# ccw1996/Paddle_hackathon

Hardware: AMD Instinct MI355X
Metric: tokens/sec GPT-3-1.3B fleet DP (bf16, whole job) (higher is better)
Workload: dtype bf16; 1 GPU; model=GPT-3-1.3B, global_batch=48, seq_len=2048, parallelism=dp1, micro_batch_per_gpu=48, n_params=1315819520, optimizer=AdamW fp32-master

## Files before the change

paddle_hackathon_amd/csrc/kernels/ce_gelu_embed.hip:

```cpp
#include "common.h"
#include <algorithm>

using namespace pha;

namespace {

template <typename T, bool VEC = true>
__global__ __launch_bounds__(256) void softmax_ce_fwd_kernel(const T* __restrict__ logits, const int64_t* __restrict__ labels,
                                                             float* __restrict__ loss, float* __restrict__ lse_out,
                                                             int V, int ignore_index) {
  const long row = blockIdx.x;
  const T* xr = logits + row * (long)V;
  float m = -INFINITY, s = 0.f;
  if constexpr (VEC) {
    for (int c = threadIdx.x * 8; c < V; c += 256 * 8) {
      float v[8];
      Vec8<T>::ld(xr + c, v);
      float vm = v[0];
#pragma unroll
      for (int i = 1; i < 8; ++i) vm = fmaxf(vm, v[i]);
      const float nm = fmaxf(m, vm);
      float acc = s * __expf(m - nm);
#pragma unroll
      for (int i = 0; i < 8; ++i) acc += __expf(v[i] - nm);
// ... 83 lines not shown
  const float e = __expf(2.f * u);
  return 1.f - 2.f * __builtin_amdgcn_rcpf(e + 1.f);
}

__device__ __forceinline__ float gelu_f(float x, bool approx) {
  if (approx) {
    const float k = 0.7978845608028654f;
    const float u = k * (x + 0.044715f * x * x * x);
    return 0.5f * x * (1.f + fast_tanh(u));
  }
  return 0.5f * x * (1.f + erff(x * 0.7071067811865476f));
}

__device__ __forceinline__ float gelu_grad(float x, bool approx) {
  if (approx) {
    constexpr float k = 0.7978845608028654f, c = 0.044715f;
    constexpr float c0 = -2.f * k * 1.4426950408889634f, c1 = c0 * c;
    const float x2 = x * x;
    const float sg = __builtin_amdgcn_rcpf(1.f + __builtin_amdgcn_exp2f(x * __builtin_fmaf(x2, c1, c0)));
    const float q = x * __builtin_fmaf(x2, 6.f * k * c, 2.f * k) * (1.f - sg);
    return __builtin_fmaf(q, sg, sg);
  }
  const float cdf = 0.5f * (1.f + erff(x * 0.7071067811865476f));
  const float pdf = 0.3989422804014327f * __expf(-0.5f * x * x);
  return cdf + x * pdf;
}

template <typename T>
__global__ __launch_bounds__(256) void bias_gelu_fwd_kernel(const T* __restrict__ x, const T* __restrict__ b, T* __restrict__ y,
                                                            long n8, int H, bool approx) {
  for (long i = blockIdx.x * 256L + threadIdx.x; i < n8; i += (long)gridDim.x * 256) {
    float v[8], o[8];
    Vec8<T>::ld(x + i * 8, v);
    if (b) {
      float bv[8];
      Vec8<T>::ld(b + (int)((unsigned)i % (unsigned)(H / 8)) * 8, bv);
// ... 585 lines not shown
```

paddle_hackathon_amd/csrc/kernels/common.h:

```cpp
#pragma once
#include <hip/hip_runtime.h>
#include <stdint.h>

#define PHA_API extern "C" __attribute__((visibility("default")))

namespace pha {

enum DType : int { kF32 = 0, kBF16 = 1, kF16 = 2 };

struct bf16_t { uint16_t v; };
struct half_t { _Float16 v; };

__device__ __forceinline__ float bf16_to_f32(uint16_t h) {
  return __uint_as_float(static_cast<uint32_t>(h) << 16);
}
__device__ __forceinline__ uint16_t f32_to_bf16(float f) {
  uint32_t u = __float_as_uint(f);
  if ((u & 0x7fffffffu) > 0x7f800000u) return 0x7fc0;
  u += 0x7fffu + ((u >> 16) & 1u);
  return static_cast<uint16_t>(u >> 16);
}

template <typename T> struct Cvt;
template <> struct Cvt<float> {
// ... 61 lines not shown
  }
};
template <> struct Vec8<float> {
  static __device__ __forceinline__ void ld(const float* p, float (&o)[8]) {
    float4 a = *reinterpret_cast<const float4*>(p);
    float4 b = *reinterpret_cast<const float4*>(p + 4);
    o[0] = a.x; o[1] = a.y; o[2] = a.z; o[3] = a.w;
    o[4] = b.x; o[5] = b.y; o[6] = b.z; o[7] = b.w;
  }
  static __device__ __forceinline__ void st(float* p, const float (&o)[8]) {
    *reinterpret_cast<float4*>(p) = make_float4(o[0], o[1], o[2], o[3]);
    *reinterpret_cast<float4*>(p + 4) = make_float4(o[4], o[5], o[6], o[7]);
  }
};

__device__ __forceinline__ float wave_sum(float v) {
#pragma unroll
  for (int o = 32; o > 0; o >>= 1) v += __shfl_xor(v, o, 64);
  return v;
}
__device__ __forceinline__ float wave_max(float v) {
#pragma unroll
  for (int o = 32; o > 0; o >>= 1) v = fmaxf(v, __shfl_xor(v, o, 64));
  return v;
}

template <bool kMax>
__device__ __forceinline__ float block_reduce(float v, float* red) {
  const int lane = threadIdx.x & 63, wid = threadIdx.x >> 6, nw = blockDim.x >> 6;
  v = kMax ? wave_max(v) : wave_sum(v);
// ... 18 lines not shown
```

paddle_hackathon_amd/csrc/kernels/gemm4p.hip:

```cpp
#include "mfma_tile.h"
#include <type_traits>

namespace pha {
namespace g4p {

using namespace g256;

#ifndef PHA_G4P_RELG_NT
#define PHA_G4P_RELG_NT 8
#endif
#ifndef PHA_G4P_CS_SPLITLOOP
#define PHA_G4P_CS_SPLITLOOP 1
#endif
#ifndef PHA_G4P_RELG_TN
#define PHA_G4P_RELG_TN 8
#endif

enum : int {
  EPI_BIAS = 1,
  EPI_GELU = 2,
  EPI_NOSTORE = 512,
  EPI_SKIP = 128,
  EPI_STAGGER = 4096,
  EPI_ROUNDS = 8192,
  EPI_TEMPORAL = 16384,
  EPI_RSTAGE = 32768,
  EPI_EARLY = 65536,
  EPI_LATE_SHIFT = 17,
  EPI_L2ONLY = 1 << 21,
  EPI_RING = 1 << 22,
  EPI_ADEEP = 1 << 23,
  EPI_WSTAG = 1 << 24,
  EPI_KSTAG_SHIFT = 25,
  EPI_COLSUM = 1 << 27,
  EPI_SPREAD_SHIFT = 28,
// ... 41 lines not shown
               :: "v"(voff), "s"(sbase), "s"(m0) : "memory", "m0");
}
__device__ __forceinline__ void glds4(const void* src, unsigned m0) {
  asm volatile("s_mov_b32 m0, %1\n\ts_nop 0\n\tglobal_load_lds_dword %0, off"
               :: "v"(src), "s"(m0) : "memory", "m0");
}

__device__ __forceinline__ void bar() {
  asm volatile("" ::: "memory");
  __builtin_amdgcn_s_barrier();
  asm volatile("" ::: "memory");
}

typedef unsigned u32x4v __attribute__((ext_vector_type(4)));

__device__ __forceinline__ float gelu_t(float x) {
  constexpr float c0 = -2.f * 0.7978845608028654f * 1.4426950408889634f;
  constexpr float c1 = c0 * 0.044715f;
  const float arg = x * __builtin_fmaf(x * x, c1, c0);
  return x * __builtin_amdgcn_rcpf(__builtin_amdgcn_exp2f(arg) + 1.f);
}

template <typename T>
__device__ __forceinline__ unsigned pk(float lo, float hi) {
  if constexpr (std::is_same<T, bf16_t>::value) {
    typedef __bf16 bf2 __attribute__((ext_vector_type(2)));
    return __builtin_bit_cast(unsigned, bf2{(__bf16)lo, (__bf16)hi});
  } else {
    typedef _Float16 h2 __attribute__((ext_vector_type(2)));
    return __builtin_bit_cast(unsigned, h2{(_Float16)lo, (_Float16)hi});
  }
}

template <typename T>
__device__ __forceinline__ void mma0(f32x4& d, const uint4& a, const uint4& b) {
// ... 26 lines not shown
    const int item = c0 + r * step;
    int lin = item / splits;
    slice = __builtin_amdgcn_readfirstlane(item - lin * splits);
    bi = __builtin_amdgcn_readfirstlane(lin / per_batch);
    lin -= bi * per_batch;
    const int group = lin / (gm * tiles_n);
    const int first_m = group * gm;
    const int gsize = min(tiles_m - first_m, gm);
    const int in = lin - group * gm * tiles_n;
    tm = __builtin_amdgcn_readfirstlane(first_m + in % gsize);
    tn = __builtin_amdgcn_readfirstlane(in / gsize);
  }
};

template <typename T, bool AKO, bool BKO, bool OT, bool BIAS, bool SKIPEPI = false, bool SPLIT = false,
          bool GELU = false, bool RS = false, bool EARLY = false, int LV = 0, bool CS = false>
__global__ __launch_bounds__(256) __attribute__((amdgpu_waves_per_eu(1, 1))) void gemm4p_kernel(Args p) {
  __shared__ __attribute__((aligned(1024))) unsigned char smem[SMEM];
  const int tid = threadIdx.x, lane = tid & 63;
  const int wid = __builtin_amdgcn_readfirstlane(tid >> 6);
  const int wr = wid >> 1, wc = wid & 1;
  const int M = p.M, N = p.N, K = p.K;
  const int nsplit = SPLIT ? p.splits : 1;
  const int nk = (K >> 6) / nsplit;

  Sched sc;
  sc.tiles_m = (M + 255) >> 8;
  sc.tiles_n = (N + 255) >> 8;
  sc.splits = nsplit;
  sc.per_batch = sc.tiles_m * sc.tiles_n;
  sc.total = sc.per_batch * nsplit * p.batch;
  sc.G = gridDim.x;
// ... 135 lines not shown
  const int lcol4 = wc * 128 + 4 * fk;
  const unsigned lane_voff4 = (unsigned)(fr * ldc2 + lcol4 * 4);
  const char* e_base = static_cast<const char*>(p.c);
  const char* e_aux = static_cast<const char*>(p.aux);
  int e_rows = 0, e_cols = 0, e_slot = 0;
  auto set_epi = [&](int r) {
    int tm, tn, slice, bi;
    sc.tile(r, tm, tn, slice, bi);
    const int r0 = OT ? tn << 8 : tm << 8, c0 = OT ? tm << 8 : tn << 8;
    e_slot = r & 3;
    if constexpr (SPLIT)
      e_base = reinterpret_cast<const char*>(p.ws) + (size_t)slice * Mo * No * 4 +
               ((size_t)(r0 + wrow) * ldc2 + (size_t)c0 * 4);
    else
      e_base = static_cast<const char*>(p.c) + (size_t)bi * p.sc * 2 + ((size_t)(r0 + wrow) * ldc2 + (size_t)c0 * 2);
    if constexpr (GELU) e_aux = static_cast<const char*>(p.aux) + ((size_t)(r0 + wrow) * ldc2 + (size_t)c0 * 2);
    e_rows = (p.epi & EPI_NOSTORE) ? 0 : Mo - r0 - wrow;
    e_cols = No - c0;
  };
  auto store_pair = [&](const f32x4& x0, const f32x4& x1, int rb, int cb) {
    float v0[4], v1[4];
    asm volatile("v_accvgpr_read_b32 %0, %4\n\tv_accvgpr_read_b32 %1, %5\n\tv_accvgpr_read_b32 %2, %6\n\t"
                 "v_accvgpr_read_b32 %3, %7"
                 : "=v"(v0[0]), "=v"(v0[1]), "=v"(v0[2]), "=v"(v0[3]) : "a"(x0[0]), "a"(x0[1]), "a"(x0[2]), "a"(x0[3]));
    asm volatile("v_accvgpr_read_b32 %0, %4\n\tv_accvgpr_read_b32 %1, %5\n\tv_accvgpr_read_b32 %2, %6\n\t"
                 "v_accvgpr_read_b32 %3, %7"
                 : "=v"(v1[0]), "=v"(v1[1]), "=v"(v1[2]), "=v"(v1[3]) : "a"(x1[0]), "a"(x1[1]), "a"(x1[2]), "a"(x1[3]));
    const int nbytes = __builtin_amdgcn_readfirstlane(max(min(e_rows - rb * 16, 16), 0) * ldc2);
    const unsigned voff = (lcol + cb * 16 < e_cols) ? lane_voff : 0x80000000u;
    typedef unsigned u32x4 __attribute__((ext_vector_type(4)));
    auto pack_swap = [&](const float (&a)[4], const float (&b)[4]) {
      unsigned q00 = pk<T>(a[0], a[1]), q01 = pk<T>(a[2], a[3]);
      unsigned q10 = pk<T>(b[0], b[1]), q11 = pk<T>(b[2], b[3]);
      const auto s0 = __builtin_amdgcn_permlane16_swap(q00, q10, false, false);
      const auto s1 = __builtin_amdgcn_permlane16_swap(q01, q11, false, false);
      return u32x4{s0[0], s1[0], s0[1], s1[1]};
    };
    auto rsrc = [&](const char* base) {
      const size_t bp = (size_t)(base + (size_t)rb * 16 * ldc2);
      const unsigned blo = __builtin_amdgcn_readfirstlane((unsigned)bp);
      const unsigned bhi = __builtin_amdgcn_readfirstlane((unsigned)(bp >> 32));
      return __builtin_amdgcn_make_buffer_rsrc(reinterpret_cast<void*>(((size_t)bhi << 32) | blo), (short)0, nbytes,
                                               0x00020000);
    };
    if constexpr (GELU)
      __builtin_amdgcn_raw_buffer_store_b128(pack_swap(v0, v1), rsrc(e_aux), voff + cb * 32, 0, 2);
    if constexpr (BIAS) {
      const unsigned char* bs = smem + BIAS_OFF + e_slot * 1024 + (OT ? wr : wc) * 512 + 16 * fk;
      const f32x4 b0 = *reinterpret_cast<const f32x4*>(bs + cb * 64);
      const f32x4 b1 = *reinterpret_cast<const f32x4*>(bs + cb * 64 + 64);
#pragma unroll
      for (int e = 0; e < 4; ++e) {
        v0[e] += b0[e];
        v1[e] += b1[e];
      }
    }
    if constexpr (GELU) {
#pragma unroll
      for (int e = 0; e < 4; ++e) {
        v0[e] = gelu_t(v0[e]);
        v1[e] = gelu_t(v1[e]);
      }
    }
    const auto rs = rsrc(e_base);
    const u32x4 q = pack_swap(v0, v1);
    if (p.epi & EPI_TEMPORAL) __builtin_amdgcn_raw_buffer_store_b128(q, rs, voff + cb * 32, 0, 0);
    else __builtin_amdgcn_raw_buffer_store_b128(q, rs, voff + cb * 32, 0, 2);
  };

  auto store_f32 = [&](const f32x4& x, int rb, int cb) {
    float v[4];
    asm volatile("v_accvgpr_read_b32 %0, %4\n\tv_accvgpr_read_b32 %1, %5\n\tv_accvgpr_read_b32 %2, %6\n\t"
// ... 50 lines not shown
        }
      }
      if constexpr (ST && RS) {
        asm volatile("s_waitcnt vmcnt(%0)" :: "n"(STV - 1) : "memory");
        stage_write(s);
        stage_load(s);
      } else if constexpr (ST) {
        stage_one(s);
      }
      const int i = s >> 1, jb = (s & 1) * 4;
      if constexpr (MODE == 2 && SPLIT) {
#pragma unroll
        for (int q = 0; q < 4; ++q) store_f32(acc[i][jb + q], i, jb + q);
      } else if constexpr (MODE == 2) {
        if constexpr (!OT) {
          store_pair(acc[i][jb], acc[i][jb + 1], i, jb);
          store_pair(acc[i][jb + 2], acc[i][jb + 3], i, jb + 2);
        } else if ((i & 1) == 0) {
#pragma unroll
          for (int q = 0; q < 4; ++q) store_pair(acc[i][jb + q], acc[i + 1][jb + q], jb + q, i);
        }
      }
#pragma unroll
      for (int q = 0; q < 4; ++q) {
        const int j = jb + q;
        if constexpr (MODE == 0) {
          if constexpr (OT) acc[i][j] = Mf<T>::mma(ca[i], cb[j], acc[i][j]);
          else acc[i][j] = Mf<T>::mma(cb[j], ca[i], acc[i][j]);
        } else {
          if constexpr (OT) mma0<T>(acc[i][j], ca[i], cb[j]);
          else mma0<T>(acc[i][j], cb[j], ca[i]);
        }
// ... 94 lines not shown
          if (s < SGB) {
#pragma unroll
            for (int d = SNA + s * (16 - SNA) / SGB; d < SNA + (s + 1) * (16 - SNA) / SGB; ++d) stage_one(d);
          }
        } else if (s < RELG) {
          if constexpr (WSTAG) dq = 16 - RELG + s;
          else stage_one(16 - RELG + s);
        }
      }
      const int i = s >> 1, jb = (s & 1) * 4;
      if constexpr (MODE == 2 && SPLIT) {
#pragma unroll
        for (int q = 0; q < 4; ++q) store_f32(acc[i][jb + q], i, jb + q);
      } else if constexpr (MODE == 2) {
        if constexpr (!OT) {
          store_pair(acc[i][jb], acc[i][jb + 1], i, jb);
          store_pair(acc[i][jb + 2], acc[i][jb + 3], i, jb + 2);
        } else if ((i & 1) == 0) {
#pragma unroll
          for (int q = 0; q < 4; ++q) store_pair(acc[i][jb + q], acc[i + 1][jb + q], jb + q, i);
        }
      }
#pragma unroll
      for (int q = 0; q < 4; ++q) {
        const int j = jb + q;
        if constexpr (WSTAG) {
          if (dq >= 0 && wid == q) stage_one(dq);
        }
        if constexpr (MODE == 0) {
          if constexpr (OT) acc[i][j] = Mf<T>::mma(ca[i], cb[j], acc[i][j]);
          else acc[i][j] = Mf<T>::mma(cb[j], ca[i], acc[i][j]);
        } else {
// ... 30 lines not shown
    for (int gi = 0; gi < 16; ++gi) stage_load(gi);
    stage_end();
  }
  asm volatile("s_waitcnt vmcnt(0)" ::: "memory");
  bar();
#pragma unroll
  for (int i = 0; i < 8; ++i) {
    fa0[i] = readA(0, 0, i);
    fb0[i] = readB(0, 0, i);
  }

#pragma unroll
  for (int i = 0; i < 8; ++i)
#pragma unroll
    for (int j = 0; j < 8; ++j) acc[i][j] = f32x4{0.f, 0.f, 0.f, 0.f};

  int s = 0;
  if constexpr (EARLY && !SKIPEPI && !RS) {
    using yes = std::true_type;
    using no = std::false_type;
    using M0 = std::integral_constant<int, 0>;
    using M2 = std::integral_constant<int, 2>;
    constexpr int NSTE = (SPLIT || GELU) ? 64 : 32;
    constexpr int VB2 = SNA + NSTE > 63 ? 63 : SNA + NSTE;
    constexpr int VL2 = 16 + NSTE > 63 ? 63 : 16 + NSTE;
    using VW1 = std::integral_constant<int, LWG ? 16 : 0>;
    using VW2 = std::integral_constant<int, LWG ? VL2 : 0>;
    const unsigned long long sp_0 = STAMP ? __builtin_amdgcn_s_memtime() : 0;
    for (int r = 0; sc.valid(r); ++r) {
      int klo = 0, khi = 0;
      if constexpr (CS) {
        int tm, tn, slice, bi;
        sc.tile(r, tm, tn, slice, bi);
        klo = __builtin_amdgcn_readfirstlane(tm * nk / sc.tiles_m);
        khi = __builtin_amdgcn_readfirstlane((tm + 1) * nk / sc.tiles_m);
      }
      using CSY = std::integral_constant<bool, CS>;
      auto sel = [&](int k, int h) -> unsigned {
// ... 2 lines not shown
      {
        const int buf = s & 1;
        phaseE(M2{}, yes{}, VW2{}, fa0, fb0, fa1, fb1, buf, 1, buf, CSY{}, sel(0, 0));
        if constexpr (LWG == 0) {
          if constexpr (STAMP) sp_t = __builtin_amdgcn_s_memtime();
          asm volatile("s_waitcnt vmcnt(%0)\n\ts_waitcnt lgkmcnt(0)" :: "n"(VB2) : "memory");
          __builtin_amdgcn_sched_barrier(0);
          bar();
          if constexpr (STAMP) {
            sp_ab += __builtin_amdgcn_s_memtime() - sp_t;
            ++sp_n;
            __builtin_amdgcn_sched_barrier(0);
          }
        }
        set_epi(r);
        phaseE(M0{}, no{}, VW2{}, fa1, fb1, fa0, fb0, buf ^ 1, 0, buf, CSY{}, sel(0, 1));
        stage_end();
        ++s;
      }
      auto ktile = [&](auto cs_c, int k) {
        const int buf = s & 1;
        phaseE(M0{}, yes{}, VW1{}, fa0, fb0, fa1, fb1, buf, 1, buf, cs_c, sel(k, 0));
        if constexpr (LWG == 0) {
          if constexpr (STAMP) sp_t = __builtin_amdgcn_s_memtime();
          asm volatile("s_waitcnt vmcnt(%0)\n\ts_waitcnt lgkmcnt(0)" :: "n"(SNA) : "memory");
          __builtin_amdgcn_sched_barrier(0);
          bar();
          if constexpr (STAMP) {
            sp_ab += __builtin_amdgcn_s_memtime() - sp_t;
            ++sp_n;
// ... 49 lines not shown
      }
    }
  } else {
  using ST1 = std::integral_constant<int, 1>;
  using STB = std::integral_constant<int, RS ? 16 : 1>;
  using STB2 = std::integral_constant<int, RS ? 16 + 32 : 1>;
  (void)sizeof(ST1);
  for (int r = 0; sc.valid(r); ++r) {
    {
      const int buf = s & 1;
      if constexpr (SKIPEPI) phase(yes{}, M1{}, M0{}, fa0, fb0, fa1, fb1, buf, 1);
      else phase(yes{}, M2{}, M0{}, fa0, fb0, fa1, fb1, buf, 1);
      static_assert(NST == 32, "vmcnt literal");
      if constexpr (RS) asm volatile("s_waitcnt lgkmcnt(0)" ::: "memory");
      else if constexpr (SPLIT || GELU) asm volatile("s_waitcnt vmcnt(63)\n\ts_waitcnt lgkmcnt(0)" ::: "memory");
      else asm volatile("s_waitcnt vmcnt(32)\n\ts_waitcnt lgkmcnt(0)" ::: "memory");
      __builtin_amdgcn_sched_barrier(0);
      bar();
      set_epi(r);
      stage_begin(buf);
      phase(yes{}, M0{}, STB2{}, fa1, fb1, fa0, fb0, buf ^ 1, 0);
      stage_end();
      ++s;
    }
    for (int k = 1; k < nk; ++k, ++s) {
      const int buf = s & 1;
      phase(yes{}, M0{}, M0{}, fa0, fb0, fa1, fb1, buf, 1);
      if constexpr (RS) asm volatile("s_waitcnt lgkmcnt(0)" ::: "memory");
      else asm volatile("s_waitcnt vmcnt(0)\n\ts_waitcnt lgkmcnt(0)" ::: "memory");
      __builtin_amdgcn_sched_barrier(0);
      bar();
      stage_begin(buf);
      phase(yes{}, M0{}, STB{}, fa1, fb1, fa0, fb0, buf ^ 1, 0);
      stage_end();
    }
  }
  }
  asm volatile("s_waitcnt vmcnt(0)" ::: "memory");
#pragma unroll
  for (int i = 0; i < 8; ++i) {
#pragma unroll
    for (int jb = 0; jb < 8; jb += 2) {
      if constexpr (SPLIT) {
        store_f32(acc[i][jb], i, jb);
        store_f32(acc[i][jb + 1], i, jb + 1);
      } else if constexpr (!OT) store_pair(acc[i][jb], acc[i][jb + 1], i, jb);
      else if ((i & 1) == 0) {
        store_pair(acc[i][jb], acc[i + 1][jb], jb, i);
        store_pair(acc[i][jb + 1], acc[i + 1][jb + 1], jb + 1, i);
      }
    }
  }
}

template <typename T, bool BIAS>
__global__ __launch_bounds__(256) void splitk_reduce_kernel(const float* __restrict__ ws, T* __restrict__ c,
                                                            const float* __restrict__ bias, int M, int N, int ldc,
                                                            int splits) {
  const long i = ((long)blockIdx.x * 256 + threadIdx.x) * 8;
  if (i >= (long)M * N) return;
  const int m = (int)(i / N), n = (int)(i - (long)m * N);
  float acc[8];
// ... 512 lines not shown
      }
    }
    if (!cs) hipLaunchKernelGGL((gemm4p_kernel<T, true, true, false, false, false, true, false, false, E>), dim3(grid), dim3(256), 0, st, a);
    const long elems = (long)a.M * a.N;
    hipLaunchKernelGGL((splitk_reduce_kernel<T, BIAS>), dim3((unsigned)((elems / 8 + 255) / 256)), dim3(256), 0, st,
                       a.ws, static_cast<T*>(a.c), a.bias, a.M, a.N, a.ldc, a.splits);
    return (int)hipGetLastError();
  }
  if constexpr (std::is_same<T, bf16_t>::value && !BIAS && !E) {
    if ((a.epi & EPI_SKIP) && !ako && !bko && !trans) {
      hipLaunchKernelGGL((gemm4p_kernel<T, false, false, false, false, true>), dim3(grid), dim3(256), 0, st, a);
      return (int)hipGetLastError();
    }
  }
  if constexpr (!BIAS) {
    if ((a.epi & EPI_ADEEP) && !(a.epi & EPI_GELU) && !ako && !bko && !trans && a.K >= 256) {
      hipLaunchKernelGGL((gemm4a_kernel<T>), dim3(grid), dim3(256), 0, st, a);
      return (int)hipGetLastError();
    }
  }
  if ((a.epi & EPI_RING) && !ako && !bko && !trans && a.K >= 128 && a.K % 64 == 0) {
    if (a.epi & EPI_GELU)
      hipLaunchKernelGGL((gemm4r_kernel<T, BIAS, true>), dim3(grid), dim3(256), 0, st, a);
    else
      hipLaunchKernelGGL((gemm4r_kernel<T, BIAS, false>), dim3(grid), dim3(256), 0, st, a);
    return (int)hipGetLastError();
  }
  if (!E && (a.epi & EPI_RSTAGE) && !ako && !bko && !trans) {
    if (a.epi & EPI_GELU)
      hipLaunchKernelGGL((gemm4p_kernel<T, false, false, false, BIAS, false, false, true, true>), dim3(grid), dim3(256), 0, st, a);
    else
      hipLaunchKernelGGL((gemm4p_kernel<T, false, false, false, BIAS, false, false, false, true>), dim3(grid), dim3(256), 0, st, a);
  } else if ((a.epi & EPI_GELU) && !ako && !bko && !trans)
    hipLaunchKernelGGL((gemm4p_kernel<T, false, false, false, BIAS, false, false, true, false, E>), dim3(grid), dim3(256), 0, st, a);
  else if (a.epi & EPI_GELU)
    return (int)hipErrorInvalidValue;
  else if (!ako && !bko && !trans) {
    const int lv = E && std::is_same<T, bf16_t>::value
                       ? ((a.epi >> EPI_LATE_SHIFT) & 15) | ((a.epi & EPI_WSTAG) ? 16 : 0) | (((a.epi >> EPI_SPREAD_SHIFT) & 3) << 5)
                       : 0;
    if (lv == 40) hipLaunchKernelGGL((gemm4p_kernel<T, false, false, false, BIAS, false, false, false, false, E, 40>), dim3(grid), dim3(256), 0, st, a);
// ... 47 lines not shown
PHA_API int pha_gemm4p_batched(int dt, const void* a, const void* b, void* c, long M, long N, long K, long lda,
                               long ldb, long ldc, int a_kouter, int b_kouter, int trans, int epi, const float* bias,
                               int grid, int group_m, float* ws, int splits, hipStream_t stream, void* aux, int batch,
                               long sa, long sb, long sc) {
  if (M <= 0 || N <= 0 || K <= 0 || K % 64 || M % 8 || N % 8 || lda % 8 || ldb % 8 || ldc % 8)
    return (int)hipErrorInvalidValue;
  if ((a_kouter && M < 8) || (b_kouter && N < 8)) return (int)hipErrorInvalidValue;
  if (M > (1L << 30) || N > (1L << 30) || K > (1L << 30) || lda > (1L << 30) || ldb > (1L << 30))
    return (int)hipErrorInvalidValue;
  if ((a_kouter ? 64.0 * lda : 256.0 * lda) * 2 >= 4294967295.0 || (b_kouter ? 64.0 * ldb : 256.0 * ldb) * 2 >= 4294967295.0)
    return (int)hipErrorInvalidValue;
  if (256.0 * ldc * 2 >= 2147483647.0) return (int)hipErrorInvalidValue;
  if (((size_t)a | (size_t)b | (size_t)c) & 15) return (int)hipErrorInvalidValue;
  if ((epi & g4p::EPI_BIAS) && !bias) return (int)hipErrorInvalidValue;
  if ((epi & g4p::EPI_GELU) && (!aux || ((size_t)aux & 15) || splits > 1)) return (int)hipErrorInvalidValue;
  if ((epi & g4p::EPI_COLSUM) && (!aux || ((size_t)aux & 3) || !a_kouter || !b_kouter || trans || batch != 1 ||
                                  !(epi & g4p::EPI_EARLY) || ((epi >> g4p::EPI_KSTAG_SHIFT) & 3) || (epi & g4p::EPI_GELU)))
    return (int)hipErrorInvalidValue;
  if (splits < 1) splits = 1;
  if (batch < 1 || (batch > 1 && (splits > 1 || (epi & g4p::EPI_GELU) || (sa | sb | sc) % 8 || sa < 0 || sb < 0 || sc < 0)))
    return (int)hipErrorInvalidValue;
  if ((double)batch * ((M + 255) / 256) * ((N + 255) / 256) >= 2147483647.0) return (int)hipErrorInvalidValue;
  if (splits > 1 && (!ws || (K / 64) % splits || !a_kouter || !b_kouter || trans || (size_t)ws & 15))
    return (int)hipErrorInvalidValue;
  const long tiles = ((M + 255) / 256) * ((N + 255) / 256) * splits * batch;
  if (grid <= 0 || grid > tiles) grid = (int)tiles;
  if (group_m <= 0) group_m = 4;
  g4p::Args p{a, b, c, bias, (int)M, (int)N, (int)K, (int)lda, (int)ldb, (int)ldc, epi, group_m, ws, splits, aux,
              batch, sa, sb, sc};
  const bool bs = epi & g4p::EPI_BIAS;
// ... 14 lines not shown
```

paddle_hackathon_amd/ops/gemm.py:

```python
from __future__ import annotations

import os
from ctypes import c_int, c_long, c_void_p

import torch

from . import _lib

EPI_BIAS, EPI_GELU, EPI_RELU, EPI_DGELU, EPI_COLSUM, EPI_AUXOUT, EPI_TRANS = 1, 2, 4, 8, 16, 32, 64
EPI_RSTAGE = 32768
EPI_EARLY = 65536
EPI_RING = 1 << 22
EPI_ADEEP = 1 << 23
EPI_WSTAG = 1 << 24
G4P_COLSUM = 1 << 27
G4P_SPREAD_SHIFT = 28
_DT = {torch.bfloat16: 1, torch.float16: 2, torch.float32: 0}


def _L():
    L = _lib._load()
    if L is None:
        raise RuntimeError(f"libpha_kernels.so not loaded: {_lib._load_error}")
    if not getattr(L, "_g4w_sig", False):
        P, I, LG = c_void_p, c_int, c_long
        L.pha_gemm4w.argtypes = [I, P, P, P, LG, LG, LG, LG, LG, LG, I, I, I, P, P, LG, P, I, P]
        L.pha_gemm4w.restype = c_int
        L.pha_gemm4p.argtypes = [I, P, P, P, LG, LG, LG, LG, LG, LG, I, I, I, I, P, I, I, P, I, P, P]
        L.pha_gemm4p.restype = c_int
# ... 85 lines not shown
    return res[0] if len(res) == 1 else tuple(res)


def _num_cus(dev):
    return torch.cuda.get_device_properties(dev).multi_processor_count


def _group_m(a_kouter, b_kouter, K, N):
    env = os.environ.get("PHA_G4P_GROUP_M")
    if env:
        return int(env)
    return 8 if (not a_kouter and not b_kouter and K < 4096 and N <= 8192) else 4


def gemm_p(a, b, a_kouter=False, b_kouter=False, bias=None, out=None, trans_out=False, epi_extra=0, grid=0,
           group_m=0, splits=1, gelu_aux=None, colsum=False):
    assert a.dtype in (torch.bfloat16, torch.float16) and b.dtype == a.dtype and a.dim() == 2 and b.dim() == 2
    assert a.stride(1) == 1 and b.stride(1) == 1
    M, Ka = (a.shape[1], a.shape[0]) if a_kouter else (a.shape[0], a.shape[1])
    N, Kb = (b.shape[1], b.shape[0]) if b_kouter else (b.shape[0], b.shape[1])
    assert Ka == Kb, (a.shape, b.shape, a_kouter, b_kouter)
    assert (a_kouter, b_kouter, trans_out) in ((False, False, False), (True, True, False), (True, False, True))
    OM, ON = (N, M) if trans_out else (M, N)
    c = out if out is not None else torch.empty(OM, ON, dtype=a.dtype, device=a.device)
    assert c.shape == (OM, ON) and c.stride(1) == 1
    epi = epi_extra | _epi_default(a_kouter, b_kouter, trans_out, Ka)
    if bias is not None:
        bias = bias.float().contiguous()
        assert bias.numel() == ON
        epi |= EPI_BIAS
    ws = None
    if splits > 1:
        ws = torch.empty(splits * OM * ON, dtype=torch.float32, device=a.device)
    if gelu_aux is not None:
        assert (a_kouter, b_kouter, trans_out, splits) == (False, False, False, 1)
        assert gelu_aux.shape == c.shape and gelu_aux.stride() == c.stride() and gelu_aux.dtype == c.dtype
        epi |= EPI_GELU
    part = None
    if colsum:
        assert (a_kouter, b_kouter, trans_out) == (True, True, False) and gelu_aux is None
        part = torch.empty(2 * splits * -(-M // 256) + 8, N, dtype=torch.float32, device=a.device)
        epi |= G4P_COLSUM | EPI_EARLY
        gelu_aux = part
    if group_m <= 0:
        group_m = _group_m(a_kouter, b_kouter, Ka, N)
    rc = _L().pha_gemm4p(_DT[a.dtype], _ptr(a), _ptr(b), _ptr(c), M, N, Ka, a.stride(0), b.stride(0), c.stride(0),
                         int(a_kouter), int(b_kouter), int(trans_out), epi, _ptr(bias), grid or _num_cus(a.device),
                         group_m, _ptr(ws), splits, _stream(a), _ptr(gelu_aux))
    if rc != 0:
        raise RuntimeError(f"pha_gemm4p failed ({rc}) M={M} N={N} K={Ka} a_kouter={a_kouter} b_kouter={b_kouter}")
    return (c, part) if colsum else c

# ... 210 lines not shown
    N = bt.shape[0]
    if _own_ok("nt", a, bt, shape=(N, K)) and bt.dtype == a.dtype:
        a, bt = _c(a), _c(bt)
        if supported(M, N, K, a, bt):
            return gemm_p(a, bt, False, False, bias=bias)
        if _own_fits(a) and _own_fits(bt):
            bp = bias if N % 8 == 0 else torch.nn.functional.pad(bias.float(), (0, -(-N // 8) * 8 - N))
            return gemm_p(_pad2(a, 8, 64), _pad2(bt, 8, 64), False, False, bias=bp)[:M, :N]
    return _lib_call("nt", "nt+bias", (M, N, K), lambda: torch.addmm(bias, a, bt.t()))


def nn(a, b, **epi):
    return gemm(b, a, True, False, trans_out=True, **epi)


def mm_nt_bias_gelu(a, bt, bias):
    M, K = a.shape
    N = bt.shape[0]
    if not (_impl() != "library" and a.is_cuda and bt.dtype == a.dtype and a.dtype in (torch.bfloat16, torch.float16)
            and supported(M, N, K, a, bt) and bias is not None and bias.numel() == N):
        return None
    pre = torch.empty(M, N, dtype=a.dtype, device=a.device)
    act = gemm_p(a, bt, False, False, bias=bias, gelu_aux=pre)
    return act, pre


def mm_nn(a, b):
    M, K = a.shape
    N = b.shape[1]
    if _own_ok("nn", a, b) and b.dtype == a.dtype:
        a, b = _c(a), _c(b)
        if supported(M, N, K, a, b):
            return nn_p(a, b)
        if _own_fits(a) and _own_fits(b):
            return nn_p(_pad2(a, 8, 64), _pad2(b, 64, 8))[:M, :N]
    return _lib_call("nn", "nn", (M, N, K), lambda: a @ b)


def mm_tn(a, b):
# ... 146 lines not shown
```

paddle_hackathon_amd/ops/mlp.py:

```python
from __future__ import annotations

import os

import torch

from . import gemm as G
from . import hip as _hip

def _eligible(x2d, w1, b1, w2, b2):
    return (x2d.is_cuda and x2d.dtype in (torch.bfloat16, torch.float16)
            and all(t is not None and t.dtype == x2d.dtype and t.is_contiguous() for t in (w1, b1, w2, b2))
            and w1.dim() == 2 and w2.dim() == 2 and w1.shape[1] == w2.shape[0] and x2d.shape[1] == w1.shape[0])


def _own_ok(x2d, w1, w2):
    M, H = x2d.shape
    F = w1.shape[1]
    return (G._own_ok("nn", x2d, w1, w2) and G.supported(F, M, H, w1, x2d) and G.supported(M, F, H, x2d, w2))


def _fwd(mode, x2d, w1, b1, approximate=True):
    if mode == 1:
        return G.nn(x2d, w1, bias=b1, act="gelu", aux_out=True)
    from .conv_gemm import weight_t
    if mode == 2:
        r = G.mm_nt_bias_gelu(x2d, weight_t(w1), b1)
        if r is not None:
            return r
    h = G.mm_nt(x2d, weight_t(w1))
    return _hip.bias_gelu_fwd(h, b1, approximate), h


def _bwd_gelu(mode, gy, w2, pre, b1, want_db=True, approximate=True):
    if mode == 1:
        g, part = G.gemm(gy, w2, False, False, act="dgelu", aux=pre, colsum=True)
        return g, G.colsum_finish(part, b1.dtype)
    ga = G.mm_nt(gy, w2)
    return _hip.bias_gelu_bwd(ga, pre, b1, approximate, want_db=want_db)


_MODES = {"pass": 0, "force": 1, "epi": 2}


def pick_mode(x2d, w1, b1, w2):
    mode = _MODES.get(os.environ.get("PHA_FUSED_MLP", _DEFAULT), 0)
    if mode == 1 and not _own_ok(x2d, w1, w2):
        return 0
    return mode


_DEFAULT = "epi"


class FusedMLP(torch.autograd.Function):
    @staticmethod
    def forward(ctx, x2d, w1, b1, w2, b2, mode, approximate=True):
        from .conv_gemm import weight_t
        a, pre = _fwd(mode, x2d, w1, b1, approximate)
        y = G.mm_nt(a, weight_t(w2)) if b2 is None else G.mm_nt_bias(a, weight_t(w2), b2)
        ctx.save_for_backward(x2d, w1, b1, w2, pre, a)
        ctx.mode, ctx.approximate = mode, approximate
        return y

    @staticmethod
    def backward(ctx, gy):
        from .conv_gemm import weight_grad
        x2d, w1, b1, w2, pre, a = ctx.saved_tensors
        gy = gy.contiguous()
        if ctx.needs_input_grad[4]:
            dw2, db2 = G.mm_tn_db(a, gy)
        else:
            dw2, db2 = weight_grad(a, gy), None
        fused_db = ctx.mode != 1
        g, db1 = _bwd_gelu(ctx.mode, gy, w2, pre, b1, want_db=not fused_db, approximate=ctx.approximate)
        dx = G.mm_nt(g, w1) if ctx.needs_input_grad[0] else None
        if fused_db:
            dw1, db1 = G.mm_tn_db(x2d, g, b1.dtype)
        else:
            dw1 = weight_grad(x2d, g)
        return dx, dw1, db1, dw2, db2, None, None


def fused_mlp(x, w1, b1, w2, b2, approximate=True):
    x2d = x.reshape(-1, x.shape[-1])
    if not x2d.is_contiguous():
        x2d = x2d.contiguous()
    mode = pick_mode(x2d, w1, b1, w2) if approximate else 0
    y = FusedMLP.apply(x2d, w1, b1, w2, b2, mode, bool(approximate))
    return y.reshape(list(x.shape[:-1]) + [w2.shape[1]])
# ... 7 lines not shown
```

Measured before the change: 128,000 tokens/s.

## Store GELU derivative in fc1 epilogue and fuse multiply into fc2 dgrad GEMM

The fc1 forward GEMM epilogue now writes the tanh-GELU derivative into the aux buffer instead of the pre-activation. In backward, the fc2 data-gradient GEMM multiplies its output by that stored derivative in its epilogue, with an aux prefetch pipeline and hand-computed vmcnt wait counts. This removes the separate bias_gelu_bwd elementwise pass over the large MLP intermediate. In exchange the forward epilogue does extra math, the MUL epilogue issues extra loads that may stall or raise register pressure, and the stored derivative is rounded to bf16.

New measurement: 129,500 tokens/s (median of 6 runs). +1.1%, better.

```diff
diff --git a/paddle_hackathon_amd/csrc/kernels/ce_gelu_embed.hip b/paddle_hackathon_amd/csrc/kernels/ce_gelu_embed.hip
--- a/paddle_hackathon_amd/csrc/kernels/ce_gelu_embed.hip
+++ b/paddle_hackathon_amd/csrc/kernels/ce_gelu_embed.hip
@@ -121,12 +121,8 @@
 
 __device__ __forceinline__ float gelu_grad(float x, bool approx) {
   if (approx) {
-    constexpr float k = 0.7978845608028654f, c = 0.044715f;
-    constexpr float c0 = -2.f * k * 1.4426950408889634f, c1 = c0 * c;
     const float x2 = x * x;
-    const float sg = __builtin_amdgcn_rcpf(1.f + __builtin_amdgcn_exp2f(x * __builtin_fmaf(x2, c1, c0)));
-    const float q = x * __builtin_fmaf(x2, 6.f * k * c, 2.f * k) * (1.f - sg);
-    return __builtin_fmaf(q, sg, sg);
+    return gelu_tanh_grad_sig(x, x2, gelu_tanh_sig(x, x2));
   }
   const float cdf = 0.5f * (1.f + erff(x * 0.7071067811865476f));
   const float pdf = 0.3989422804014327f * __expf(-0.5f * x * x);
diff --git a/paddle_hackathon_amd/csrc/kernels/common.h b/paddle_hackathon_amd/csrc/kernels/common.h
--- a/paddle_hackathon_amd/csrc/kernels/common.h
+++ b/paddle_hackathon_amd/csrc/kernels/common.h
@@ -99,6 +99,17 @@
   }
 };
 
+__device__ __forceinline__ float gelu_tanh_sig(float x, float x2) {
+  constexpr float k = 0.7978845608028654f, c = 0.044715f;
+  constexpr float c0 = -2.f * k * 1.4426950408889634f, c1 = c0 * c;
+  return __builtin_amdgcn_rcpf(1.f + __builtin_amdgcn_exp2f(x * __builtin_fmaf(x2, c1, c0)));
+}
+__device__ __forceinline__ float gelu_tanh_grad_sig(float x, float x2, float sg) {
+  constexpr float k = 0.7978845608028654f, c = 0.044715f;
+  const float q = x * __builtin_fmaf(x2, 6.f * k * c, 2.f * k) * (1.f - sg);
+  return __builtin_fmaf(q, sg, sg);
+}
+
 __device__ __forceinline__ float wave_sum(float v) {
 #pragma unroll
   for (int o = 32; o > 0; o >>= 1) v += __shfl_xor(v, o, 64);
diff --git a/paddle_hackathon_amd/csrc/kernels/gemm4p.hip b/paddle_hackathon_amd/csrc/kernels/gemm4p.hip
--- a/paddle_hackathon_amd/csrc/kernels/gemm4p.hip
+++ b/paddle_hackathon_amd/csrc/kernels/gemm4p.hip
@@ -19,6 +19,8 @@
 enum : int {
   EPI_BIAS = 1,
   EPI_GELU = 2,
+  EPI_GELU_DAUX = 4,
+  EPI_MULAUX = 8,
   EPI_NOSTORE = 512,
   EPI_SKIP = 128,
   EPI_STAGGER = 4096,
@@ -90,11 +92,30 @@
 
 typedef unsigned u32x4v __attribute__((ext_vector_type(4)));
 
-__device__ __forceinline__ float gelu_t(float x) {
-  constexpr float c0 = -2.f * 0.7978845608028654f * 1.4426950408889634f;
-  constexpr float c1 = c0 * 0.044715f;
-  const float arg = x * __builtin_fmaf(x * x, c1, c0);
-  return x * __builtin_amdgcn_rcpf(__builtin_amdgcn_exp2f(arg) + 1.f);
+__device__ __forceinline__ float gelu_t(float x) { return x * gelu_tanh_sig(x, x * x); }
+
+constexpr int mul_dmas(int a, int b, int DF) { return b - (a > DF ? a : DF) + 1 > 0 ? b - (a > DF ? a : DF) + 1 : 0; }
+constexpr int mul_loads(int a, int b, int W) { return ((b < 15 - W ? b : 15 - W) - a + 1 > 0) ? 2 * ((b < 15 - W ? b : 15 - W) - a + 1) : 0; }
+constexpr int mul_younger(int s, int W, int PB, int DF) {
+  const int n = s >= W ? 2 * (W - 1) + mul_dmas(s - W + 1, s, DF) + mul_loads(s - W + 1, s - 1, W)
+                       : 2 * (W - 1) + PB + mul_dmas(0, s, DF) + mul_loads(0, s - 1, W);
+  return n > 63 ? 63 : n;
+}
+static_assert(mul_younger(15, 6, 8, 8) == 10 + 6 && mul_younger(0, 6, 8, 8) == 10 + 8 && mul_younger(7, 6, 0, 16) == 10 + 10,
+              "mul_younger");
+constexpr int vmcnt_imm(int n) { return (n & 15) | ((n >> 4) << 14) | (7 << 4) | (15 << 8); }
+
+template <typename T>
+__device__ __forceinline__ void unpk(unsigned q, float& lo, float& hi) {
+  if constexpr (std::is_same<T, bf16_t>::value) {
+    lo = __builtin_bit_cast(float, q << 16);
+    hi = __builtin_bit_cast(float, q & 0xffff0000u);
+  } else {
+    typedef _Float16 h2 __attribute__((ext_vector_type(2)));
+    const h2 h = __builtin_bit_cast(h2, q);
+    lo = (float)h[0];
+    hi = (float)h[1];
+  }
 }
 
 template <typename T>
@@ -151,8 +172,12 @@
 };
 
 template <typename T, bool AKO, bool BKO, bool OT, bool BIAS, bool SKIPEPI = false, bool SPLIT = false,
-          bool GELU = false, bool RS = false, bool EARLY = false, int LV = 0, bool CS = false>
+          bool GELU = false, bool RS = false, bool EARLY = false, int LV = 0, bool CS = false, bool DAUX = false,
+          bool MUL = false>
 __global__ __launch_bounds__(256) __attribute__((amdgpu_waves_per_eu(1, 1))) void gemm4p_kernel(Args p) {
+  static_assert(!DAUX || (GELU && BIAS), "the derivative aux is a variant of the bias + GELU epilogue");
+  static_assert(!MUL || !(AKO || BKO || OT || BIAS || SPLIT || GELU || RS || CS || SKIPEPI), "MUL: the plain NT build only");
+  static_assert(!MUL || (lv_lwg(LV) == 0 && !lv_wstag(LV) && !lv_stamp(LV)), "MUL: the wait counts assume these DMA placements");
   __shared__ __attribute__((aligned(1024))) unsigned char smem[SMEM];
   const int tid = threadIdx.x, lane = tid & 63;
   const int wid = __builtin_amdgcn_readfirstlane(tid >> 6);
@@ -318,11 +343,39 @@
                ((size_t)(r0 + wrow) * ldc2 + (size_t)c0 * 4);
     else
       e_base = static_cast<const char*>(p.c) + (size_t)bi * p.sc * 2 + ((size_t)(r0 + wrow) * ldc2 + (size_t)c0 * 2);
-    if constexpr (GELU) e_aux = static_cast<const char*>(p.aux) + ((size_t)(r0 + wrow) * ldc2 + (size_t)c0 * 2);
+    if constexpr (GELU || MUL) e_aux = static_cast<const char*>(p.aux) + ((size_t)(r0 + wrow) * ldc2 + (size_t)c0 * 2);
     e_rows = (p.epi & EPI_NOSTORE) ? 0 : Mo - r0 - wrow;
     e_cols = No - c0;
   };
-  auto store_pair = [&](const f32x4& x0, const f32x4& x1, int rb, int cb) {
+  constexpr int MW = 8;
+  u32x4v aw[MUL ? 2 * MW : 2];
+  auto aux_load = [&](int li) {
+    const int g = li >> 1, rb = g >> 1, cb = (g & 1) * 4 + (li & 1) * 2;
+    const size_t bp = (size_t)(e_aux + (size_t)rb * 16 * ldc2);
+    u32x4v rs;
+    rs[0] = __builtin_amdgcn_readfirstlane((unsigned)bp);
+    rs[1] = __builtin_amdgcn_readfirstlane((unsigned)(bp >> 32)) & 0xffffu;
+    rs[2] = (unsigned)__builtin_amdgcn_readfirstlane(max(min(e_rows - rb * 16, 16), 0) * ldc2);
+    rs[3] = 0x00020000u;
+    const unsigned voff = (lcol + cb * 16 < e_cols) ? lane_voff : 0x80000000u;
+    asm volatile("buffer_load_dwordx4 %0, %1, %2, 0 offen offset:%3"
+                 : "=v"(aw[MUL ? li % (2 * MW) : 0]) : "v"(voff), "s"(rs), "i"(cb * 32) : "memory");
+  };
+  auto aux_wait = [&](int s, int PB, int DF) {
+    asm volatile("s_waitcnt %2" : "+v"(aw[MUL ? (2 * s) % (2 * MW) : 0]), "+v"(aw[MUL ? (2 * s + 1) % (2 * MW) : 1])
+                 : "i"(vmcnt_imm(mul_younger(s, MW, PB, DF))) : "memory");
+  };
+  auto aux_next = [&](int s) {
+    if (s + MW < 16) {
+      aux_load(2 * (s + MW));
+      aux_load(2 * (s + MW) + 1);
+    }
+  };
+  auto aux_prefetch = [&]() {
+#pragma unroll
+    for (int li = 0; li < 2 * MW; ++li) aux_load(li);
+  };
+  auto store_pair = [&](const f32x4& x0, const f32x4& x1, int rb, int cb, int li = 0) {
     float v0[4], v1[4];
     asm volatile("v_accvgpr_read_b32 %0, %4\n\tv_accvgpr_read_b32 %1, %5\n\tv_accvgpr_read_b32 %2, %6\n\t"
                  "v_accvgpr_read_b32 %3, %7"
@@ -347,7 +400,22 @@
       return __builtin_amdgcn_make_buffer_rsrc(reinterpret_cast<void*>(((size_t)bhi << 32) | blo), (short)0, nbytes,
                                                0x00020000);
     };
-    if constexpr (GELU)
+    if constexpr (MUL) {
+      const u32x4v w = aw[MUL ? li % (2 * MW) : 0];
+      const auto t0 = __builtin_amdgcn_permlane16_swap(w[0], w[2], false, false);
+      const auto t1 = __builtin_amdgcn_permlane16_swap(w[1], w[3], false, false);
+      float m0[4], m1[4];
+      unpk<T>(t0[0], m0[0], m0[1]);
+      unpk<T>(t1[0], m0[2], m0[3]);
+      unpk<T>(t0[1], m1[0], m1[1]);
+      unpk<T>(t1[1], m1[2], m1[3]);
+#pragma unroll
+      for (int e = 0; e < 4; ++e) {
+        v0[e] *= m0[e];
+        v1[e] *= m1[e];
+      }
+    }
+    if constexpr (GELU && !DAUX)
       __builtin_amdgcn_raw_buffer_store_b128(pack_swap(v0, v1), rsrc(e_aux), voff + cb * 32, 0, 2);
     if constexpr (BIAS) {
       const unsigned char* bs = smem + BIAS_OFF + e_slot * 1024 + (OT ? wr : wc) * 512 + 16 * fk;
@@ -359,7 +427,28 @@
         v1[e] += b1[e];
       }
     }
-    if constexpr (GELU) {
+    if constexpr (DAUX) {
+      unsigned qd[4];
+#pragma unroll
+      for (int h = 0; h < 2; ++h) {
+        float da[2], db[2];
+#pragma unroll
+        for (int e2 = 0; e2 < 2; ++e2) {
+          const int e = 2 * h + e2;
+          const float a = v0[e], a2 = a * a, sa = gelu_tanh_sig(a, a2);
+          const float b = v1[e], b2 = b * b, sb = gelu_tanh_sig(b, b2);
+          da[e2] = gelu_tanh_grad_sig(a, a2, sa);
+          db[e2] = gelu_tanh_grad_sig(b, b2, sb);
+          v0[e] = a * sa;
+          v1[e] = b * sb;
+        }
+        qd[h] = pk<T>(da[0], da[1]);
+        qd[2 + h] = pk<T>(db[0], db[1]);
+      }
+      const auto s0 = __builtin_amdgcn_permlane16_swap(qd[0], qd[2], false, false);
+      const auto s1 = __builtin_amdgcn_permlane16_swap(qd[1], qd[3], false, false);
+      __builtin_amdgcn_raw_buffer_store_b128(u32x4{s0[0], s1[0], s0[1], s1[1]}, rsrc(e_aux), voff + cb * 32, 0, 2);
+    } else if constexpr (GELU) {
 #pragma unroll
       for (int e = 0; e < 4; ++e) {
         v0[e] = gelu_t(v0[e]);
@@ -440,8 +529,10 @@
         for (int q = 0; q < 4; ++q) store_f32(acc[i][jb + q], i, jb + q);
       } else if constexpr (MODE == 2) {
         if constexpr (!OT) {
-          store_pair(acc[i][jb], acc[i][jb + 1], i, jb);
-          store_pair(acc[i][jb + 2], acc[i][jb + 3], i, jb + 2);
+          if constexpr (MUL) aux_wait(s, 16, 16);
+          store_pair(acc[i][jb], acc[i][jb + 1], i, jb, 2 * s);
+          store_pair(acc[i][jb + 2], acc[i][jb + 3], i, jb + 2, 2 * s + 1);
+          if constexpr (MUL) aux_next(s);
         } else if ((i & 1) == 0) {
 #pragma unroll
           for (int q = 0; q < 4; ++q) store_pair(acc[i][jb + q], acc[i + 1][jb + q], jb + q, i);
@@ -566,8 +657,10 @@
         for (int q = 0; q < 4; ++q) store_f32(acc[i][jb + q], i, jb + q);
       } else if constexpr (MODE == 2) {
         if constexpr (!OT) {
-          store_pair(acc[i][jb], acc[i][jb + 1], i, jb);
-          store_pair(acc[i][jb + 2], acc[i][jb + 3], i, jb + 2);
+          if constexpr (MUL) aux_wait(s, 16 - SNA, RELG);
+          store_pair(acc[i][jb], acc[i][jb + 1], i, jb, 2 * s);
+          store_pair(acc[i][jb + 2], acc[i][jb + 3], i, jb + 2, 2 * s + 1);
+          if constexpr (MUL) aux_next(s);
         } else if ((i & 1) == 0) {
 #pragma unroll
           for (int q = 0; q < 4; ++q) store_pair(acc[i][jb + q], acc[i + 1][jb + q], jb + q, i);
@@ -628,6 +721,10 @@
   for (int i = 0; i < 8; ++i)
 #pragma unroll
     for (int j = 0; j < 8; ++j) acc[i][j] = f32x4{0.f, 0.f, 0.f, 0.f};
+  if constexpr (MUL) {
+#pragma unroll
+    for (int i = 0; i < 2 * MW; ++i) aw[i] = u32x4v{0u, 0u, 0u, 0u};
+  }
 
   int s = 0;
   if constexpr (EARLY && !SKIPEPI && !RS) {
@@ -635,7 +732,8 @@
     using no = std::false_type;
     using M0 = std::integral_constant<int, 0>;
     using M2 = std::integral_constant<int, 2>;
-    constexpr int NSTE = (SPLIT || GELU) ? 64 : 32;
+    static_assert(!MUL || (RELG == 8 && SNA == 8), "MUL: one DMA per group from RELG on (mul_younger)");
+    constexpr int NSTE = (SPLIT || GELU) ? 64 : MUL ? 64 - 2 * MW : 32;
     constexpr int VB2 = SNA + NSTE > 63 ? 63 : SNA + NSTE;
     constexpr int VL2 = 16 + NSTE > 63 ? 63 : 16 + NSTE;
     using VW1 = std::integral_constant<int, LWG ? 16 : 0>;
@@ -668,6 +766,7 @@
           }
         }
         set_epi(r);
+        if constexpr (MUL) aux_prefetch();
         phaseE(M0{}, no{}, VW2{}, fa1, fb1, fa0, fb0, buf ^ 1, 0, buf, CSY{}, sel(0, 1));
         stage_end();
         ++s;
@@ -747,10 +846,12 @@
       static_assert(NST == 32, "vmcnt literal");
       if constexpr (RS) asm volatile("s_waitcnt lgkmcnt(0)" ::: "memory");
       else if constexpr (SPLIT || GELU) asm volatile("s_waitcnt vmcnt(63)\n\ts_waitcnt lgkmcnt(0)" ::: "memory");
+      else if constexpr (MUL) asm volatile("s_waitcnt vmcnt(%0)\n\ts_waitcnt lgkmcnt(0)" :: "n"(64 - 2 * MW) : "memory");
       else asm volatile("s_waitcnt vmcnt(32)\n\ts_waitcnt lgkmcnt(0)" ::: "memory");
       __builtin_amdgcn_sched_barrier(0);
       bar();
       set_epi(r);
+      if constexpr (MUL) aux_prefetch();
       stage_begin(buf);
       phase(yes{}, M0{}, STB2{}, fa1, fb1, fa0, fb0, buf ^ 1, 0);
       stage_end();
@@ -777,8 +878,15 @@
       if constexpr (SPLIT) {
         store_f32(acc[i][jb], i, jb);
         store_f32(acc[i][jb + 1], i, jb + 1);
-      } else if constexpr (!OT) store_pair(acc[i][jb], acc[i][jb + 1], i, jb);
-      else if ((i & 1) == 0) {
+      } else if constexpr (!OT) {
+        if constexpr (MUL) {
+          if ((jb & 3) == 0) aux_wait(2 * i + (jb >> 2), 0, 16);
+        }
+        store_pair(acc[i][jb], acc[i][jb + 1], i, jb, 4 * i + (jb >> 1));
+        if constexpr (MUL) {
+          if ((jb & 3) == 2) aux_next(2 * i + (jb >> 2));
+        }
+      } else if ((i & 1) == 0) {
         store_pair(acc[i][jb], acc[i + 1][jb], jb, i);
         store_pair(acc[i][jb + 1], acc[i + 1][jb + 1], jb + 1, i);
       }
@@ -1321,7 +1429,7 @@
     }
   }
   if constexpr (!BIAS) {
-    if ((a.epi & EPI_ADEEP) && !(a.epi & EPI_GELU) && !ako && !bko && !trans && a.K >= 256) {
+    if ((a.epi & EPI_ADEEP) && !(a.epi & (EPI_GELU | EPI_MULAUX)) && !ako && !bko && !trans && a.K >= 256) {
       hipLaunchKernelGGL((gemm4a_kernel<T>), dim3(grid), dim3(256), 0, st, a);
       return (int)hipGetLastError();
     }
@@ -1332,6 +1440,20 @@
     else
       hipLaunchKernelGGL((gemm4r_kernel<T, BIAS, false>), dim3(grid), dim3(256), 0, st, a);
     return (int)hipGetLastError();
+  }
+  if constexpr (BIAS) {
+    if (a.epi & EPI_GELU_DAUX) {
+      if (!E && (a.epi & EPI_RSTAGE))
+        hipLaunchKernelGGL((gemm4p_kernel<T, false, false, false, true, false, false, true, true, false, 0, false, true>), dim3(grid), dim3(256), 0, st, a);
+      else
+        hipLaunchKernelGGL((gemm4p_kernel<T, false, false, false, true, false, false, true, false, E, 0, false, true>), dim3(grid), dim3(256), 0, st, a);
+      return (int)hipGetLastError();
+    }
+  } else {
+    if (a.epi & EPI_MULAUX) {
+      hipLaunchKernelGGL((gemm4p_kernel<T, false, false, false, false, false, false, false, false, E, E ? 40 : 0, false, false, true>), dim3(grid), dim3(256), 0, st, a);
+      return (int)hipGetLastError();
+    }
   }
   if (!E && (a.epi & EPI_RSTAGE) && !ako && !bko && !trans) {
     if (a.epi & EPI_GELU)
@@ -1409,6 +1531,15 @@
   if (((size_t)a | (size_t)b | (size_t)c) & 15) return (int)hipErrorInvalidValue;
   if ((epi & g4p::EPI_BIAS) && !bias) return (int)hipErrorInvalidValue;
   if ((epi & g4p::EPI_GELU) && (!aux || ((size_t)aux & 15) || splits > 1)) return (int)hipErrorInvalidValue;
+  if (epi & (g4p::EPI_GELU_DAUX | g4p::EPI_MULAUX)) {
+    if (a_kouter || b_kouter || trans || splits > 1 || batch != 1 || !aux || ((size_t)aux & 15) ||
+        (epi & (g4p::EPI_COLSUM | g4p::EPI_RING)))
+      return (int)hipErrorInvalidValue;
+    if ((epi & g4p::EPI_GELU_DAUX) && ((epi & g4p::EPI_MULAUX) || !(epi & g4p::EPI_GELU) || !(epi & g4p::EPI_BIAS)))
+      return (int)hipErrorInvalidValue;
+    if ((epi & g4p::EPI_MULAUX) && (epi & (g4p::EPI_GELU | g4p::EPI_BIAS | g4p::EPI_RSTAGE)))
+      return (int)hipErrorInvalidValue;
+  }
   if ((epi & g4p::EPI_COLSUM) && (!aux || ((size_t)aux & 3) || !a_kouter || !b_kouter || trans || batch != 1 ||
                                   !(epi & g4p::EPI_EARLY) || ((epi >> g4p::EPI_KSTAG_SHIFT) & 3) || (epi & g4p::EPI_GELU)))
     return (int)hipErrorInvalidValue;
diff --git a/paddle_hackathon_amd/ops/gemm.py b/paddle_hackathon_amd/ops/gemm.py
--- a/paddle_hackathon_amd/ops/gemm.py
+++ b/paddle_hackathon_amd/ops/gemm.py
@@ -13,6 +13,8 @@
 EPI_RING = 1 << 22
 EPI_ADEEP = 1 << 23
 EPI_WSTAG = 1 << 24
+G4P_GELU_DAUX = 4
+G4P_MULAUX = 8
 G4P_COLSUM = 1 << 27
 G4P_SPREAD_SHIFT = 28
 _DT = {torch.bfloat16: 1, torch.float16: 2, torch.float32: 0}
@@ -128,7 +130,7 @@
 
 
 def gemm_p(a, b, a_kouter=False, b_kouter=False, bias=None, out=None, trans_out=False, epi_extra=0, grid=0,
-           group_m=0, splits=1, gelu_aux=None, colsum=False):
+           group_m=0, splits=1, gelu_aux=None, colsum=False, gelu_deriv=False, mul_aux=None):
     assert a.dtype in (torch.bfloat16, torch.float16) and b.dtype == a.dtype and a.dim() == 2 and b.dim() == 2
     assert a.stride(1) == 1 and b.stride(1) == 1
     M, Ka = (a.shape[1], a.shape[0]) if a_kouter else (a.shape[0], a.shape[1])
@@ -150,6 +152,17 @@
         assert (a_kouter, b_kouter, trans_out, splits) == (False, False, False, 1)
         assert gelu_aux.shape == c.shape and gelu_aux.stride() == c.stride() and gelu_aux.dtype == c.dtype
         epi |= EPI_GELU
+        if gelu_deriv:
+            assert bias is not None, "the derivative aux is a variant of the bias + GELU epilogue"
+            epi |= G4P_GELU_DAUX
+    else:
+        assert not gelu_deriv
+    if mul_aux is not None:
+        assert (a_kouter, b_kouter, trans_out, splits) == (False, False, False, 1)
+        assert gelu_aux is None and bias is None and not colsum
+        assert mul_aux.shape == c.shape and mul_aux.stride() == c.stride() and mul_aux.dtype == c.dtype
+        epi |= G4P_MULAUX
+        gelu_aux = mul_aux
     part = None
     if colsum:
         assert (a_kouter, b_kouter, trans_out) == (True, True, False) and gelu_aux is None
@@ -390,15 +403,29 @@
     return gemm(b, a, True, False, trans_out=True, **epi)
 
 
-def mm_nt_bias_gelu(a, bt, bias):
+def mm_nt_bias_gelu(a, bt, bias, deriv=False):
     M, K = a.shape
     N = bt.shape[0]
     if not (_impl() != "library" and a.is_cuda and bt.dtype == a.dtype and a.dtype in (torch.bfloat16, torch.float16)
             and supported(M, N, K, a, bt) and bias is not None and bias.numel() == N):
         return None
     pre = torch.empty(M, N, dtype=a.dtype, device=a.device)
-    act = gemm_p(a, bt, False, False, bias=bias, gelu_aux=pre)
+    act = gemm_p(a, bt, False, False, bias=bias, gelu_aux=pre, gelu_deriv=deriv)
     return act, pre
+
+
+def mm_nt_mul(a, bt, aux, out=None):
+    M, K = a.shape
+    N = bt.shape[0]
+    if not (_impl() != "library" and a.is_cuda and bt.dtype == a.dtype and a.dtype in (torch.bfloat16, torch.float16)
+            and aux.dtype == a.dtype and tuple(aux.shape) == (M, N) and supported(M, N, K, a, bt, aux)):
+        return None
+    if out is None:
+        out = torch.empty_strided((M, N), aux.stride(), dtype=a.dtype, device=a.device)
+    elif not (out.dtype == a.dtype and tuple(out.shape) == (M, N) and out.stride() == aux.stride()
+              and supported(M, N, K, out)):
+        return None
+    return gemm_p(a, bt, False, False, out=out, mul_aux=aux)
 
 
 def mm_nn(a, b):
diff --git a/paddle_hackathon_amd/ops/mlp.py b/paddle_hackathon_amd/ops/mlp.py
--- a/paddle_hackathon_amd/ops/mlp.py
+++ b/paddle_hackathon_amd/ops/mlp.py
@@ -19,27 +19,38 @@
     return (G._own_ok("nn", x2d, w1, w2) and G.supported(F, M, H, w1, x2d) and G.supported(M, F, H, x2d, w2))
 
 
-def _fwd(mode, x2d, w1, b1, approximate=True):
+def _fwd(mode, x2d, w1, b1, approximate=True, w2=None):
     if mode == 1:
-        return G.nn(x2d, w1, bias=b1, act="gelu", aux_out=True)
+        return G.nn(x2d, w1, bias=b1, act="gelu", aux_out=True) + (False,)
     from .conv_gemm import weight_t
-    if mode == 2:
+    if mode == 3 and w2 is not None and G.supported(x2d.shape[0], w2.shape[0], w2.shape[1], w2):
+        r = G.mm_nt_bias_gelu(x2d, weight_t(w1), b1, deriv=True)
+        if r is not None:
+            return r + (True,)
+    if mode in (2, 3):
         r = G.mm_nt_bias_gelu(x2d, weight_t(w1), b1)
         if r is not None:
-            return r
+            return r + (False,)
     h = G.mm_nt(x2d, weight_t(w1))
-    return _hip.bias_gelu_fwd(h, b1, approximate), h
+    return _hip.bias_gelu_fwd(h, b1, approximate), h, False
 
 
-def _bwd_gelu(mode, gy, w2, pre, b1, want_db=True, approximate=True):
+def _bwd_gelu(mode, gy, w2, pre, b1, want_db=True, approximate=True, deriv=False):
     if mode == 1:
         g, part = G.gemm(gy, w2, False, False, act="dgelu", aux=pre, colsum=True)
         return g, G.colsum_finish(part, b1.dtype)
+    if deriv:
+        g = G.mm_nt_mul(gy, w2, pre)
+        if g is None:
+            from . import fallback
+            fallback.note("fused_mlp", "fc2 dgrad x stored GELU derivative outside the own kernel")
+            g = G.mm_nt(gy, w2).mul_(pre)
+        return g, (_hip.col_sum(g, b1.dtype) if want_db else None)
     ga = G.mm_nt(gy, w2)
     return _hip.bias_gelu_bwd(ga, pre, b1, approximate, want_db=want_db)
 
 
-_MODES = {"pass": 0, "force": 1, "epi": 2}
+_MODES = {"pass": 0, "force": 1, "epi": 2, "epi2": 3}
 
 
 def pick_mode(x2d, w1, b1, w2):
@@ -49,17 +60,17 @@
     return mode
 
 
-_DEFAULT = "epi"
+_DEFAULT = "epi2"
 
 
 class FusedMLP(torch.autograd.Function):
     @staticmethod
     def forward(ctx, x2d, w1, b1, w2, b2, mode, approximate=True):
         from .conv_gemm import weight_t
-        a, pre = _fwd(mode, x2d, w1, b1, approximate)
+        a, pre, deriv = _fwd(mode, x2d, w1, b1, approximate, w2)
         y = G.mm_nt(a, weight_t(w2)) if b2 is None else G.mm_nt_bias(a, weight_t(w2), b2)
         ctx.save_for_backward(x2d, w1, b1, w2, pre, a)
-        ctx.mode, ctx.approximate = mode, approximate
+        ctx.mode, ctx.approximate, ctx.deriv = mode, approximate, deriv
         return y
 
     @staticmethod
@@ -72,7 +83,8 @@
         else:
             dw2, db2 = weight_grad(a, gy), None
         fused_db = ctx.mode != 1
-        g, db1 = _bwd_gelu(ctx.mode, gy, w2, pre, b1, want_db=not fused_db, approximate=ctx.approximate)
+        g, db1 = _bwd_gelu(ctx.mode, gy, w2, pre, b1, want_db=not fused_db, approximate=ctx.approximate,
+                           deriv=ctx.deriv)
         dx = G.mm_nt(g, w1) if ctx.needs_input_grad[0] else None
         if fused_db:
             dw1, db1 = G.mm_tn_db(x2d, g, b1.dtype)
```
